# pingooio/pingoo

Hardware: AMD Instinct MI355X
Metric: requests/sec matched (whole node), 1k-rule WAF (higher is better)
Workload: dtype u8

## Files before the change

pingoo_amd/csrc/confirm.hip:

```cpp
#include <hip/hip_runtime.h>

#include <algorithm>

#include "confirm.h"
#include "hitrec.h"
#include "kernels.h"
#include "wave.h"

namespace pwaf {

__global__ __launch_bounds__(256) void confirm_plan_kernel(ConfirmTableDev b, uint32_t *plan ) {
    __shared__ uint32_t part[256];
    const uint32_t t = threadIdx.x;
    uint32_t items = 0;
    if (t < b.count) {
        const ConfirmArgs *pa = &b.c[t];
        const bool dense = pa->dense_flag != nullptr && *pa->dense_flag > pa->dense_thresh;
        items = dense ? 0u : (min(*pa->pair_count, pa->pair_cap) + kConfirmThreads - 1) / kConfirmThreads;
    }
    part[t] = items;
    __syncthreads();
    for (uint32_t d = 1; d < 256; d <<= 1) {
        const uint32_t v = t >= d ? part[t - d] : 0u;
        __syncthreads();
        part[t] += v;
        __syncthreads();
    }
    if (t < b.count) plan[t] = part[t] - items;
    if (t == 0) plan[b.count] = part[255];
}

__device__ __noinline__ void merge_atom(PoolEntry *pool, uint32_t *pool_count, uint32_t *status, uint32_t pool_cap, uint32_t *rec, uint32_t atom) {
    auto rmw_read = [](uint32_t *p) { return atomicOr(p, 0u); };
    auto publish = [&](uint32_t idx, uint32_t at, uint32_t next) {
        const uint32_t t0 = atomicExch(&pool[idx].atom, at), t1 = atomicExch(&pool[idx].next, next);
        asm volatile("" ::"v"(t0), "v"(t1));
    };
    uint32_t old = rmw_read(rec);
    for (;;) {
        uint32_t upd;
        const uint32_t x = atom + 1u;
        if (!(old & REC_OVERFLOW)) {
            const uint32_t a0 = old & 0x7FFFu, a1 = (old >> 15) & 0x7FFFu;
            if (a0 == x || a1 == x) return;
            if (a0 == 0u) upd = old | x;
            else if (a1 == 0u) upd = old | (x << 15);
            else {
                const uint32_t idx = atomicAdd(pool_count, 3u);
                if (idx + 3u > pool_cap) { atomicOr(status, 1u); return; }
                publish(idx, a0 - 1u, kNone);
                publish(idx + 1u, a1 - 1u, idx);
                publish(idx + 2u, atom, idx + 1u);
                upd = REC_OVERFLOW | (idx + 2u);
            }
        } else {
            const uint32_t head = old & ~REC_OVERFLOW;
            for (uint32_t i = head; i != kNone; i = rmw_read(&pool[i].next))
                if (rmw_read(&pool[i].atom) == atom) return;
            const uint32_t idx = atomicAdd(pool_count, 1u);
            if (idx >= pool_cap) { atomicOr(status, 1u); return; }
            publish(idx, atom, head);
            upd = REC_OVERFLOW | idx;
        }
        const uint32_t seen = atomicCAS(rec, old, upd);
        if (seen == old) return;
        old = seen;
    }
}

__global__ __launch_bounds__(kConfirmThreads, 8) void confirm_kernel(ConfirmTableDev b, const uint32_t *plan) {
    __shared__ uint32_t head[kFilterEntries], ftab[kFilterEntries];
    __shared__ uint32_t pool[kConfirmPoolBytes / 4];
    constexpr uint32_t kConfirmQueue = 1024;
    __shared__ uint32_t app_cnt, app_base, app_queue[kConfirmQueue];
    __builtin_amdgcn_s_setprio(3);
    if (threadIdx.x == 0) app_cnt = 0;
    const uint32_t total = plan[b.count];
    const uint32_t it0 = (uint32_t)((uint64_t)total * blockIdx.x / gridDim.x), it1 = (uint32_t)((uint64_t)total * (blockIdx.x + 1) / gridDim.x);
    for (uint32_t it = it0; it < it1;) {
        uint32_t ps = 0;
        for (uint32_t lo = 0, hi = b.count; lo + 1 < hi;) {
            const uint32_t mid = (lo + hi) >> 1;
            if (plan[mid] <= it) lo = mid;
            else hi = mid;
            ps = lo;
        }
        const uint32_t first_item = plan[ps], it_end = min(it1, plan[ps + 1]);
        const ConfirmArgs a = load_descriptor(&b.c[ps]);
        __syncthreads();
        {
            const uint4 *sh = reinterpret_cast<const uint4 *>(a.c_head), *sf = reinterpret_cast<const uint4 *>(a.ftable);
            constexpr uint32_t kPer = kFilterEntries / 4 / kConfirmThreads;
            uint4 vh[kPer], vf[kPer];
#pragma unroll
            for (uint32_t q = 0; q < kPer; q++) { vh[q] = sh[q * kConfirmThreads + threadIdx.x]; vf[q] = sf[q * kConfirmThreads + threadIdx.x]; }
#pragma unroll
            for (uint32_t q = 0; q < kPer; q++) {
                reinterpret_cast<uint4 *>(head)[q * kConfirmThreads + threadIdx.x] = vh[q];
                reinterpret_cast<uint4 *>(ftab)[q * kConfirmThreads + threadIdx.x] = vf[q];
            }
        }
        const uint32_t e_words = a.n_entries * 3u, b_words = a.n_bytes / 4u, c_words = a.n_class_words;
        const bool in_lds = confirm_tables_fit(a.n_entries, a.n_bytes, a.n_class_words);
        const ConfirmEntry *t_entries = a.c_entries;
        const uint8_t *t_bytes = a.c_bytes;
        const uint32_t *t_classes = a.c_classes;
        if (in_lds) {
            const uint32_t *se = reinterpret_cast<const uint32_t *>(a.c_entries), *sb = reinterpret_cast<const uint32_t *>(a.c_bytes);
            for (uint32_t k = threadIdx.x; k < e_words; k += kConfirmThreads) pool[k] = se[k];
            for (uint32_t k = threadIdx.x; k < b_words; k += kConfirmThreads) pool[e_words + k] = sb[k];
            for (uint32_t k = threadIdx.x; k < c_words; k += kConfirmThreads) pool[e_words + b_words + k] = a.c_classes[k];
            t_entries = reinterpret_cast<const ConfirmEntry *>(pool);
            t_bytes = reinterpret_cast<const uint8_t *>(pool + e_words);
            t_classes = pool + e_words + b_words;
        }
        __syncthreads();
        const ConfirmView cv{nullptr, t_entries, t_bytes, t_classes, a.mul, a.stride, a.init};
        const uint32_t n_p = min(*a.pair_count, a.pair_cap);
        auto pair_of = [&](const uint32_t item) -> uint2 {
            const uint32_t k = (item - first_item) * kConfirmThreads + threadIdx.x;
            return (item < it_end && k < n_p) ? a.pairs[k] : make_uint2(kNone, 0u);
        };
        uint2 pr_next = pair_of(it), pr_after = pair_of(it + 1u);
        uint32_t fs_next = 0u, fe_next = 0u;
        ConfirmBytes tb_next{};
        if (pr_next.x != kNone) {
            confirm_load64(reinterpret_cast<const uint8_t *>(a.off + pr_next.x), fs_next, fe_next);
            tb_next = confirm_chunk_bytes(a.data, pr_next.y, a.total + PWAF_ARENA_PAD);
        }
        for (; it < it_end; it++) {
            const uint2 pr = pr_next;
            const bool live = pr.x != kNone;
            uint32_t r = live ? pr.x : 0u;
            uint32_t fs = fs_next, fe = fe_next;
            const ConfirmBytes tb = tb_next;
            pr_next = pr_after;
            if (pr_next.x != kNone) {
                confirm_load64(reinterpret_cast<const uint8_t *>(a.off + pr_next.x), fs_next, fe_next);
                tb_next = confirm_chunk_bytes(a.data, pr_next.y, a.total + PWAF_ARENA_PAD);
            }
            pr_after = pair_of(it + 2u);
            ConfirmChunk ch{0u, 0ull};
            if (live) ch = confirm_windows_of(cv, tb, 0u, 0xFFFFFFFFu, pr.y, [&](const uint32_t bin) { return ftab[bin]; });
            uint32_t mask = ch.mask, cnt = 0, j = 0, e0 = 0, pos = 0, widx = 0;
            bool walk = false;
            auto settle = [&](const uint32_t rq, const uint32_t need_lits, const bool wk, const bool aggregated) -> bool {
                bool w2 = wk;
                if (need_lits & a.shared_bits) w2 = true;
                const uint32_t direct = need_lits & ~a.shared_bits;
                if (direct) enqueue_mask_once(a.gate_lists, a.gate_count, a.n, rq, direct, a.enq_bits, a.enq_words);
                if (!w2 || a.walk_list == nullptr) return false;
                const uint32_t bit = 1u << (rq & 31u);
                if (atomicOr(&a.walk_bits[rq >> 5], bit) & bit) return false;
                atomicOr(&a.valid_bits[rq >> 5], bit);
                if (aggregated) return true;
                a.walk_list[atomicAdd(a.walk_count, 1u)] = rq;
                return false;
            };
            uint32_t need = 0;
            for (;;) {
                if (__ballot(j < cnt || mask != 0u) == 0) break;
                while (j >= cnt && mask != 0u) {
                    const uint32_t k = (uint32_t)__builtin_ctz(mask);
                    mask &= mask - 1u;
                    pos = pr.y * 16u + k;
                    const uint32_t bin = confirm_bin_of(ch, widx++, a.data, pos, a.mul);
                    while (pos >= fe && r + 1u < a.n) {
                        settle(r, need, walk, false);
                        need = 0;
                        walk = false;
                        r++;
                        fs = fe;
                        fe = a.off[r + 1];
                    }
                    if (pos >= fe) continue;
                    const uint32_t hd = head[bin];
                    e0 = hd & 0xFFFFFu;
                    cnt = hd >> 20;
                    j = 0;
                }
                if (j < cnt) {
                    const uint32_t res = in_lds ? confirm_entry<3>(t_entries, t_bytes, t_classes, e0 + j, a.data, fs, fe, pos)
                                                : confirm_entry<1>(t_entries, t_bytes, t_classes, e0 + j, a.data, fs, fe, pos);
                    j++;
                    if (res == 2u) {
                        walk = true;
                    } else if (res & 1u) {
                        const uint32_t atom = res >> 8;
                        merge_atom(a.pool, a.pool_count, a.status, a.pool_cap, a.rec + r, atom);
                        atomicOr(&a.valid_bits[r >> 5], 1u << (r & 31u));
                        if (a.colmask_local != nullptr) need |= a.colmask_local[atom];
                    }
                }
            }
            const bool append = live && settle(r, need, walk, true);
            if (append) {
                const uint32_t slot = atomicAdd(&app_cnt, 1u);
                if (slot < kConfirmQueue) app_queue[slot] = r;
                else a.walk_list[atomicAdd(a.walk_count, 1u)] = r;
            }
        }
        __syncthreads();
        {
            const uint32_t queued = min(app_cnt, kConfirmQueue);
            if (threadIdx.x == 0 && queued != 0) app_base = atomicAdd(a.walk_count, queued);
            __syncthreads();
            for (uint32_t k = threadIdx.x; k < queued; k += kConfirmThreads) a.walk_list[app_base + k] = app_queue[k];
            __syncthreads();
            if (threadIdx.x == 0) app_cnt = 0;
        }
    }
}

int launch_confirm(const ConfirmArgs *host, uint32_t count, const ConfirmArgs *dev, uint32_t *plan, uint32_t n_cus, void *stream) {
    if (count == 0 || host[0].n == 0) return 0;
    if (count > 256) return (int)hipErrorInvalidValue;
    ConfirmTableDev b{dev, count};
    hipLaunchKernelGGL(confirm_plan_kernel, dim3(1), dim3(256), 0, (hipStream_t)stream, b, plan);
    hipError_t e = hipGetLastError();
    if (e != hipSuccess) return (int)e;
    uint64_t max_items = 0;
    for (uint32_t k = 0; k < count; k++) max_items += ((uint64_t)host[k].pair_cap + kConfirmThreads - 1) / kConfirmThreads;
    const uint32_t blocks = (uint32_t)std::min<uint64_t>(max_items, (uint64_t)std::max(1u, n_cus) * 2u);
    const uint32_t *cplan = plan;
    hipLaunchKernelGGL(confirm_kernel, dim3(blocks), dim3(kConfirmThreads), 0, (hipStream_t)stream, b, cplan);
    return (int)hipGetLastError();
}

}
```

pingoo_amd/csrc/engine.cpp:

```cpp
#include "dirtable.h"
#include "engine_impl.h"
#include "georec.h"

using namespace pwaf;

namespace {

Switches read_switches() {
    Switches s;
#ifdef PWAF_PROFILING
    const auto set = [](const char *name) { return getenv(name) != nullptr; };
    s.sync_each = set("PWAF_SYNC_EACH");
    if (set("PWAF_DEBUG_SKIP")) s.debug_skip = (uint32_t)strtoul(getenv("PWAF_DEBUG_SKIP"), nullptr, 0);
    s.attr_prio = set("PWAF_ATTR_PRIO");
    s.placement = set("PWAF_PLACEMENT") ? atoi(getenv("PWAF_PLACEMENT")) : set("PWAF_ATTR_INLINE") ? 1 : set("PWAF_ATTR_EARLY") ? 3 : 2;
    s.skip_attr = set("PWAF_SKIP_ATTR");
    s.skip_ipres = set("PWAF_SKIP_IPRES") || s.skip_attr;
    if (set("PWAF_LIST_SHAPE")) s.list_shape = (long)(uint32_t)atoi(getenv("PWAF_LIST_SHAPE"));
    if (set("PWAF_FILTER_DEBUG_SKIP")) s.filter_debug_skip = (uint32_t)atoi(getenv("PWAF_FILTER_DEBUG_SKIP"));
    s.attr_after_compact = set("PWAF_ATTR_AFTER_COMPACT");
    s.dump_counts = set("PWAF_DUMP_COUNTS");
    s.skip_identity = set("PWAF_SKIP_IDENTITY");
    s.side_priority_high = set("PWAF_SIDE_PRIORITY_HIGH");
    s.no_packed_staging = set("PWAF_NO_PACKED_STAGING");
#endif
    return s;
}

int upload_tables(pwaf_engine *e, const TablePlan &t) {
    const Program &P = *e->prog.p;
    int rc = PWAF_OK;
    const auto up = [&](DevBuf &buf, const auto &vec) { if (!rc) rc = upload(buf, vec); };
    static_cast<PlanShape &>(*e) = t;
    for (int var = 0; var < 2; var++) {
        up(e->iu_vals[var], t.iu_vals[var]);
        up(e->iu_masks[var], t.iu_masks[var]);
    }
    up(e->bit_atoms, t.bit_col);
    up(e->num_atoms, t.cmp_atoms);
    up(e->lazy_atoms, t.lazy_atoms);
    up(e->lits, t.lits);
    up(e->trig_off, t.trig_off);
    up(e->trig_rules, t.trig_rules);
    up(e->always_rules, t.always);
    up(e->country_luts, t.cc_masks);
    up(e->rules, P.rules);
    if (!t.rules_unrouted.empty()) up(e->rules_unrouted, t.rules_unrouted);
    up(e->set_masks, P.set_masks);
    up(e->ip_root4, P.ipset_trie.root4);
    up(e->ip_root6, P.ipset_trie.root6);
    up(e->ip_nodes, P.ipset_trie.nodes);
    up(e->class_rows, t.class_rows);
    up(e->geo_root4, t.geo_root4);
    up(e->geo_root6, t.geo_root6);
    up(e->geo_nodes, t.geo_nodes);
    up(e->leaf_root, std::vector<uint32_t>(65536, TRIE_LEAF));
    up(e->geo_leaf_root, std::vector<uint32_t>(65536, TRIE_LEAF | t.geo_default));
    if (P.n_residual) {
        up(e->residual_blob, P.residual_blob);
        up(e->residual_errors, std::vector<unsigned long long>(P.n_residual, 0ull));
        if (P.has_geo && P.residual_needs_geo) {
            const std::vector<uint32_t> leaf0(65536, TRIE_LEAF);
            up(e->geo_rec_root4, P.geo_trie.root4.empty() ? leaf0 : P.geo_trie.root4);
            up(e->geo_rec_root6, P.geo_trie.root6.empty() ? leaf0 : P.geo_trie.root6);
            up(e->geo_rec_nodes, P.geo_trie.nodes);
            up(e->geo_recs, P.geo_recs);
        }
    }
    return rc;
}

int upload_flat(FlatDev &d, const FlatImage &m) {
    int rc = PWAF_OK;
    const auto up = [&](DevBuf &buf, const auto &vec, size_t pad = 0) { if (!rc) rc = upload(buf, vec, pad); };
    static_cast<FlatShape &>(d) = m;
    up(d.flat, m.flat, 16);
    up(d.delta, m.delta, 16);
    up(d.flat_classmap, m.classmap);
    up(d.emit_off, m.emit_off);
    up(d.emit_list, m.emit_list);
    up(d.end_off, m.end_off);
    up(d.end_list, m.end_list);
    return rc;
}
int upload_group(pwaf_engine *e, size_t k, const TuneOut *T) {
    const Program &P = *e->prog.p;
    const DfaGroup &g = P.groups[k];
    DevGroup &d = e->groups[k];
    int rc;
    ScanImage m;
    if ((rc = build_device_group(g, P.lds_hot_budget, m, T ? &T->visits[k] : nullptr, T ? &T->class_freq[k] : nullptr))) return rc;
    static_cast<ScanShape &>(d) = m;
    if ((rc = upload(d.tab, m.tab, 16)) || (rc = upload(d.classmap, m.classmap)) || (rc = upload(d.special, m.special)) || (rc = upload(d.list_off, m.list_off)) ||
        (rc = upload(d.list, m.list)))
        return rc;
    FlatImage fm, rm;
    const uint32_t lds[2] = {flat_lds_bytes(false), flat_lds_bytes(true)};
    build_flat_images(g, d.filter, lds, T, k, fm, rm);
    if ((rc = upload_flat(d.fl, fm)) || !g.rtier) return rc;
    return upload_flat(d.rt, rm);
}

int assign_lists(pwaf_engine *e) {
    const Program &P = *e->prog.p;
    std::vector<GroupFilter> filters;
    for (const DevGroup &d : e->groups) filters.push_back(d.filter);
    PassPlan plan;
    plan_passes(P, filters, e->mean_len, e->residual_jit.function != nullptr, switches().skip_identity, plan);
    static_cast<PassShape &>(*e) = plan;
    std::vector<FlatShape> full, rtier;
    for (const DevGroup &d : e->groups) {
        full.push_back(d.fl);
        rtier.push_back(d.rt);
    }
    plan_list_scans(plan.roles, full, rtier, !(P.flags & PWAF_OPT_NO_DENSE_SWITCH), switches().skip_identity, switches().list_shape, e->list_plan);
    int rc = PWAF_OK;
    const auto up = [&](DevBuf &buf, const auto &vec) { if (!rc) rc = upload(buf, vec); };
    for (size_t k = 0; k < e->groups.size(); k++) {
        DevGroup &d = e->groups[k];
        static_cast<PassRole &>(d) = plan.roles[k];
        if (!d.filtered) continue;
        up(d.ftable, d.filter.table);
        if (!d.confirm) continue;
        const ConfirmTable &ct = d.filter.confirm;
        up(d.c_head, ct.head);
        up(d.c_entries, ct.entries);
        up(d.c_bytes, ct.bytes);
        up(d.c_classes, ct.classes);
    }
    if (!plan.short_atoms.empty()) up(e->short_atoms, plan.short_atoms);
    up(e->pass_table, plan.pass_table);
    up(e->colmask, plan.colmask);
    return rc;
}

}

namespace pwaf {

const Switches &switches() {
    static const Switches sw = read_switches();
    return sw;
}

void set_trie_args(const pwaf_engine *e, VerdictArgs &v) {
    const Program &P = *e->prog.p;
    const uint32_t *leaf = (const uint32_t *)e->leaf_root.p;
    v.ip_root4 = P.ipset_trie.root4.empty() ? leaf : (const uint32_t *)e->ip_root4.p;
    v.ip_root6 = P.ipset_trie.root6.empty() ? leaf : (const uint32_t *)e->ip_root6.p;
    v.ip_nodes = (const uint32_t *)e->ip_nodes.p;
    v.set_masks = (const uint32_t *)e->set_masks.p;
    v.set_words = P.set_words;
    v.n_ip_lists = P.n_ip_lists;
    const uint32_t *geo_leaf = (const uint32_t *)e->geo_leaf_root.p;
    v.geo_root4 = P.geo_trie.root4.empty() ? geo_leaf : (const uint32_t *)e->geo_root4.p;
    v.geo_root6 = P.geo_trie.root6.empty() ? geo_leaf : (const uint32_t *)e->geo_root6.p;
    v.geo_nodes = (const uint32_t *)e->geo_nodes.p;
    v.has_geo = P.has_geo ? 1u : 0u;
    v.dir24 = (const uint32_t *)e->dir24.p;
    v.dir_chunks = (const uint32_t *)e->dir_chunks.p;
    v.dir_vals = (const uint32_t *)e->dir_vals.p;
    v.dir_esc = (const uint2 *)e->dir_esc.p;
    v.dir_summary = (const uint32_t *)e->dir_summary.p;
    v.dir_sum_shift = e->dir_sum_shift;
    v.dir_common = e->dir_common;
    v.dir_coarse = (const uint32_t *)e->dir_coarse.p;
    v.dir_coarse_shift = e->dir_coarse_shift;
    v.dir_coarse_bytes = e->dir_coarse_bytes;
    v.class_rows = (const uint32_t *)e->class_rows.p;
    v.class_words = e->class_words;
    v.acmp_words = e->acmp_words;
    v.geo_default = e->geo_default;
// ... 360 lines not shown
```

pingoo_amd/csrc/engine_impl.h:

```cpp
#pragma once
#include <hip/hip_runtime_api.h>

#include <cstdio>
#include <algorithm>
#include <cstring>
#include <memory>
#include <mutex>
#include <string>
#include <vector>

#include "kernels.h"
#include "program_handle.h"
#include "scanplan.h"
#include "staging.h"
#include "tableplan.h"

#define HIP_TRY(expr)                                                                                              \
    do {                                                                                                           \
        hipError_t _e = (expr);                                                                                    \
        if (_e != hipSuccess) return pwaf::fail(PWAF_E_DEVICE, std::string(#expr) + ": " + hipGetErrorString(_e)); \
    } while (0)

#pragma GCC visibility push(hidden)
namespace pwaf {

struct Switches {
    bool sync_each = false;
    uint32_t debug_skip = 0;
    bool attr_prio = false;
    int placement = 2;
    bool skip_ipres = false;
    bool skip_attr = false;
    long list_shape = -1;
    uint32_t filter_debug_skip = 0;
    bool attr_after_compact = false;
    bool dump_counts = false;
    bool skip_identity = false;
    bool side_priority_high = false;
    bool no_packed_staging = false;
};
const Switches &switches();

struct DevBuf {
    void *p = nullptr;
    size_t cap = 0;
    DevBuf() = default;
    DevBuf(const DevBuf &) = delete;
    DevBuf &operator=(const DevBuf &) = delete;
    DevBuf(DevBuf &&o) noexcept : p(o.p), cap(o.cap) { o.p = nullptr; o.cap = 0; }
    DevBuf &operator=(DevBuf &&o) noexcept {
        if (this != &o) { release(); p = o.p; cap = o.cap; o.p = nullptr; o.cap = 0; }
        return *this;
    }
    ~DevBuf() { release(); }
    int reserve(size_t bytes) {
        if (bytes <= cap) return PWAF_OK;
        if (p) (void)hipFree(p);
        p = nullptr;
        cap = 0;
        size_t want = bytes + bytes / 8 + 256;
        hipError_t e = hipMalloc(&p, want);
        if (e != hipSuccess) return fail(PWAF_E_NOMEM, std::string("hipMalloc failed: ") + hipGetErrorString(e));
        cap = want;
        return PWAF_OK;
    }
    void release() {
        if (p) (void)hipFree(p);
        p = nullptr;
        cap = 0;
    }
};

struct PinBuf {
    void *p = nullptr;
    size_t cap = 0;
    PinBuf() = default;
    PinBuf(const PinBuf &) = delete;
    PinBuf &operator=(const PinBuf &) = delete;
    PinBuf(PinBuf &&o) noexcept : p(o.p), cap(o.cap) { o.p = nullptr; o.cap = 0; }
    PinBuf &operator=(PinBuf &&o) noexcept {
        if (this != &o) { release(); p = o.p; cap = o.cap; o.p = nullptr; o.cap = 0; }
        return *this;
    }
    ~PinBuf() { release(); }
    int reserve(size_t bytes) {
        if (bytes <= cap) return PWAF_OK;
        if (p) (void)hipHostFree(p);
        p = nullptr;
        cap = 0;
        size_t want = bytes + bytes / 4 + 4096;
        hipError_t e = hipHostMalloc(&p, want, hipHostMallocPortable);
        if (e != hipSuccess) return fail(PWAF_E_NOMEM, std::string("hipHostMalloc failed: ") + hipGetErrorString(e));
        cap = want;
        return PWAF_OK;
    }
    void release() {
        if (p) (void)hipHostFree(p);
        p = nullptr;
        cap = 0;
    }
};

template <class T>
int upload(DevBuf &b, const std::vector<T> &v, size_t pad_bytes = 0) {
    size_t bytes = v.size() * sizeof(T);
    int rc = b.reserve(bytes + pad_bytes + 16);
    if (rc) return rc;
    if (bytes) HIP_TRY(hipMemcpy(b.p, v.data(), bytes, hipMemcpyHostToDevice));
    if (pad_bytes + 16) HIP_TRY(hipMemset((char *)b.p + bytes, 0, pad_bytes + 16));
    return PWAF_OK;
}

struct FlatDev : FlatShape {
    DevBuf flat, flat_classmap, emit_off, emit_list, end_off, end_list, delta;
};

struct DevGroup : ScanShape, PassRole {
    DevBuf tab, classmap, special, list_off, list;
    uint32_t chunks = 1;
    GroupFilter filter;
    DevBuf ftable;
    FlatDev fl, rt;
    DevBuf c_head, c_entries, c_bytes, c_classes;
};

}

struct Scratch {
    using DevBuf = pwaf::DevBuf;
    using PinBuf = pwaf::PinBuf;
    std::mutex mu;
    hipStream_t stream = nullptr, side = nullptr;
    hipEvent_t ev_fork = nullptr, ev_join = nullptr, done = nullptr;
    bool used = false;
    hipStream_t last = nullptr;
    bool last_own = false;
    DevBuf status;
    uint64_t pool_entries = 0;
    struct View { void *p = nullptr; };
    View res_cols;
    bool retry = false;
    DevBuf err_sink;
    DevBuf ipres;
    DevBuf rec, pool, gate_lists, attr;
    DevBuf verdict_spill;
    DevBuf res_words;
    DevBuf zero_block;
    View ctrl, cand_bits, visit_bits, walk_bits;
    DevBuf chunk_bits, cand_cnt;
    DevBuf need;
    DevBuf pairs;
    DevBuf zero_off;
    static constexpr uint32_t kArgSlots = 8;
    DevBuf args;
    PinBuf arg_slot[kArgSlots];
    hipEvent_t arg_ev[kArgSlots] = {};
    bool arg_pending[kArgSlots] = {};
    uint32_t arg_next = 0;
    std::vector<DevBuf> stage_field_data, stage_field_off;
    DevBuf stage_ip, stage_v6, stage_port, stage_flags, stage_asn, stage_country, stage_out, stage_counts;
    DevBuf stage_route;
    DevBuf stage_hits, stage_hit_counts;
    DevBuf stage_geo;
    PinBuf pin_in, pin_out, pin_status;
    DevBuf packed;
    DevBuf rec_meta, rec_cols;
    PinBuf rec_pin, rec_back;
    int ensure(bool own_stream) {
        if (!side) {
            int least = 0, greatest = 0;
            (void)hipDeviceGetStreamPriorityRange(&least, &greatest);
            if (pwaf::switches().side_priority_high) least = greatest;
            if (hipStreamCreateWithPriority(&side, hipStreamNonBlocking, least) != hipSuccess || hipEventCreateWithFlags(&ev_fork, hipEventDisableTiming) != hipSuccess ||
                hipEventCreateWithFlags(&ev_join, hipEventDisableTiming) != hipSuccess || hipEventCreateWithFlags(&done, hipEventDisableTiming) != hipSuccess)
                return pwaf::fail(PWAF_E_DEVICE, "hipStreamCreate / hipEventCreate failed");
            for (hipEvent_t &ev : arg_ev)
                if (hipEventCreateWithFlags(&ev, hipEventDisableTiming) != hipSuccess) return pwaf::fail(PWAF_E_DEVICE, "hipEventCreate failed");
        }
        if (own_stream && !stream && hipStreamCreateWithFlags(&stream, hipStreamNonBlocking) != hipSuccess) return pwaf::fail(PWAF_E_DEVICE, "hipStreamCreate failed");
        return PWAF_OK;
    }
    ~Scratch() {
        for (hipEvent_t ev : arg_ev)
            if (ev) (void)hipEventDestroy(ev);
        if (stream) (void)hipStreamDestroy(stream);
        if (side) (void)hipStreamDestroy(side);
        for (hipEvent_t ev : {ev_fork, ev_join, done})
// ... 163 lines not shown
```

pingoo_amd/csrc/kernels.h:

```cpp
#pragma once
#include <cstdint>
#include <string>
#include <vector>

#include "program.h"
#include "scanplan.h"
#include "verdictplan.h"

namespace pwaf {

static constexpr int kMaxPasses = 250;
static constexpr int kVerdictPre = 12;
static constexpr uint32_t kDirChunkWords = 32;

static constexpr uint32_t REC_OVERFLOW = 0x80000000u;
struct PoolEntry {
    uint32_t atom;
    uint32_t next;
};

struct ScanArgs {
    const uint8_t *data;
    const uint32_t *off;
    uint32_t n;
    const uint16_t *tab;
    const uint8_t *classmap;
    const uint8_t *umap;
    uint32_t ill_class;
    const SpecialCell *special;
    const uint32_t *list_off;
    const uint16_t *list;
    uint32_t n_states, stride, n_classes, n_hot;
    uint32_t start_emit;
    uint32_t emit_base, special_base;
    uint32_t n_cus;
    uint32_t chunks;
    uint32_t *rec;
    PoolEntry *pool;
    uint32_t *pool_count;
    uint32_t pool_cap;
    uint32_t *status;
    const uint32_t *colmask_local;
    uint32_t n_local;
    uint32_t *gate_lists;
    uint32_t *gate_count;
};

static constexpr uint32_t kListWalks = 1;
struct ListScanArgs {
    const uint8_t *data;
    const uint32_t *off;
    uint32_t n;
    const uint16_t *flat;
    const uint8_t *classmap;
    const uint8_t *umap;
    uint32_t ill_class;
    uint32_t n_classes;
    uint32_t n_hot;
    const uint64_t *delta;
    uint32_t n_delta;
    const uint32_t *emit_off;
    const uint16_t *emit_list;
    const uint32_t *end_off;
    const uint16_t *end_list;
    uint32_t *rec;
    PoolEntry *pool;
    uint32_t *pool_count;
    uint32_t pool_cap;
    uint32_t *status;
    const uint32_t *colmask_local;
    uint32_t n_local;
    uint32_t *gate_lists;
    uint32_t *gate_count;
    uint32_t *enq_bits;
    uint32_t enq_words;
    uint32_t behind_filter;
    const uint32_t *req_list;
    const uint32_t *n_list;
    uint32_t *visited;
    uint32_t *need_out;
    uint32_t shared_bits;
    const uint32_t *need_in;
    uint32_t need_bit;
    uint32_t merge_rec;
    uint32_t n_cus;
    const uint32_t *dense_flag;
    uint32_t dense_thresh;
    uint32_t dense_mode;
};
struct ListOf {
    const uint32_t *req_list;
    uint32_t n_l;
};

struct ConfirmArgs {
    const uint8_t *data;
    const uint32_t *off;
    uint32_t n;
    uint32_t total;
    const uint2 *pairs;
    const uint32_t *pair_count;
    uint32_t pair_cap;
    uint32_t mul, stride, init;
    const uint32_t *ftable;
    const uint32_t *c_head;
    const ConfirmEntry *c_entries;
    const uint8_t *c_bytes;
    const uint32_t *c_classes;
    uint32_t n_entries, n_bytes, n_class_words;
    uint32_t *rec;
    uint32_t *valid_bits;
    uint32_t *walk_bits;
    uint32_t *walk_list;
    uint32_t *walk_count;
    PoolEntry *pool;
    uint32_t *pool_count;
    uint32_t pool_cap;
    uint32_t *status;
    const uint32_t *colmask_local;
    uint32_t n_local;
    uint32_t *gate_lists;
    uint32_t *gate_count;
    uint32_t *enq_bits;
    uint32_t enq_words;
    uint32_t shared_bits;
    const uint32_t *dense_flag;
    uint32_t dense_thresh;
};
static constexpr uint32_t kConfirmThreads = 1024;
static constexpr uint32_t kConfirmPoolBytes = 40 * 1024;
constexpr uint32_t confirm_table_bytes(const size_t pool_bytes) { return (uint32_t)pool_bytes & ~3u; }
constexpr bool confirm_tables_fit(const uint32_t n_entries, const uint32_t n_bytes, const uint32_t n_class_words) {
    return (uint64_t)n_entries * 3u + n_bytes / 4u + n_class_words <= kConfirmPoolBytes / 4;
}
struct ConfirmTableDev {
    const ConfirmArgs *c;
    uint32_t count;
};
int launch_confirm(const ConfirmArgs *host, uint32_t count, const ConfirmArgs *dev, uint32_t *plan, uint32_t n_cus, void *stream);

static constexpr uint32_t kStreamSlab = 128 * 1024;
static constexpr uint32_t kStreamIter = 4096;
static constexpr uint32_t kFilterWaves = 4;
static constexpr uint32_t kCompactWords = 2048;
struct FilterArgs {
    const uint8_t *data;
    const uint32_t *off;
    uint32_t n;
    uint32_t total;
    uint32_t slab0;
    uint32_t init;
    uint32_t mul;
    uint32_t stride;
    const uint32_t *table;
    uint32_t n_heads;
    uint32_t head_w[2][4];
    uint32_t head_m[2][4];
    uint32_t head_len[2];
    uint32_t head_code[2];
    uint32_t *rec;
    uint32_t *chunk_bits;
    uint32_t *sub_count;
    uint32_t *bitmap;
    uint32_t *block_count;
    uint32_t *list;
    uint32_t *list_count;
    uint2 *pairs;
    uint32_t *pair_count;
    uint32_t pair_cap;
    uint32_t *pair_base;
    const uint32_t *dense_flag;
    uint32_t dense_thresh;
    uint32_t first_block;
    uint32_t debug;
};
int upload_args_block(const void *host_pinned, void *dev, size_t bytes, void *zero , size_t zero_bytes, void *stream);
struct FilterTable {
    const FilterArgs *f;
    uint32_t count;
};
struct FilterMix {
    const FilterArgs *f1, *f2;
    uint32_t count1, count2, blocks1, blocks2;
};
int launch_filter(const FilterArgs *host1, uint32_t count1, const FilterArgs *dev1, const FilterArgs *host2, uint32_t count2, const FilterArgs *dev2, void *stream);
int launch_resolve(const FilterArgs *host, uint32_t count, const FilterArgs *dev, void *stream);
int launch_compact(const FilterArgs *host, uint32_t count, const FilterArgs *dev, void *stream);
int configure_kernels(int device);
int configure_scan_kernels();
int configure_filter_kernels();
int configure_verdict_kernels();

struct FcmpArgs {
    const uint8_t *data[kMaxFcmpFields];
    const uint32_t *off[kMaxFcmpFields];
    uint32_t atoms[kMaxFcmpAtoms];
    uint32_t n, n_atoms;
    uint32_t *rec;
    PoolEntry *pool;
    uint32_t *pool_count;
    uint32_t pool_cap;
    uint32_t *status;
};
int launch_fcmp(const FcmpArgs &a, void *stream);
struct ResidualArgs {
    const uint8_t *const *data;
    const uint32_t *const *off;
    const uint8_t *blob;
    uint32_t n, n_rules;
    const uint8_t *ip;
    const uint8_t *ip_is_v6;
    const uint16_t *port;
    const uint32_t *asn;
    const uint16_t *country;
    uint32_t has_geo;
    const uint32_t *geo_root4, *geo_root6, *geo_nodes;
    const GeoRec *geo_recs;
    uint32_t *rec;
    PoolEntry *pool;
    uint32_t *pool_count;
    uint32_t pool_cap;
    uint32_t *status;
    unsigned long long *rule_errors;
};
int launch_residual(const ResidualArgs &a, void *stream);
struct ResidualJitArgs {
    const uint8_t *const *data;
    const uint32_t *const *off;
    const uint8_t *blob;
    uint32_t n, n_rules;
    const uint8_t *ip;
    const uint8_t *ip_is_v6;
    const uint16_t *port;
    const uint32_t *asn;
    const uint16_t *country;
    uint32_t has_geo, pad;
    const uint32_t *geo_root4, *geo_root6, *geo_nodes;
    const GeoRec *geo_recs;
    uint32_t *match_words;
    unsigned long long *rule_errors;
};
struct JitKernel {
    void *module = nullptr, *function = nullptr;
};
static constexpr uint32_t kMaxJitRules = 256;
bool rvm_specialize(const uint8_t *blob, size_t len, std::string &out, std::string &why);
bool rvm_jit_program(const uint8_t *blob, size_t len, std::string &out, std::string &why);
bool rtc_compile(const std::string &source, const std::string &arch, std::vector<char> &code, std::string &why);
bool jit_load(const std::vector<char> &code, JitKernel &out, std::string &why);
void jit_release(JitKernel &k);
int launch_residual_jit(const JitKernel &k, const ResidualJitArgs &a, uint32_t n_cus, void *stream);
struct ColPtrChunk {
    const void *p[2 * (PWAF_N_FIELDS + kMaxHeaders)];
    uint32_t count;
};
struct VerdictArgs {
    uint32_t n, n_groups;
    uint32_t debug_skip;
    uint32_t force_global_tables;
    uint32_t sparse_mode;
    uint32_t v_cap;
    unsigned long long *spill;
    const uint32_t *off[PWAF_N_FIELDS];
    const uint8_t *ip;
    const uint8_t *ip_is_v6;
    const uint16_t *port;
    const uint8_t *flags;
    const uint32_t *asn;
    const uint16_t *country;
    uint32_t n_passes;
    const uint32_t *rec;
    const PassInfo *passes;
    const uint32_t *res_match;
    uint32_t res_words, res_base;
    const uint32_t *cand_bits, *visit_bits;
    uint32_t bit_words;
    const uint32_t *hoff[kMaxHeaderLens];
    const ShortAtom *short_atoms;
    uint32_t n_short;
    const uint8_t *short_data;
    const uint32_t *short_off;
    uint32_t n_hlen;
    const PoolEntry *pool;
    uint32_t n_cols;
    const CmpAtomDev *cmp;
    uint32_t n_cmp;
    uint32_t cmp_vars;
    const CmpAtomDev *lazy;
    uint32_t n_lazy;
    uint32_t lazy_var[4], n_lazy_var;
    const uint32_t *bit_col;
    const int64_t *iu_vals[2];
// ... 78 lines not shown
```

pingoo_amd/csrc/pipeline.cpp:

```cpp
#include <type_traits>

#include "engine_impl.h"
#include "georec.h"
#include "lscan_split.h"

using namespace pwaf;

namespace {

uint32_t slab_count(uint32_t total, uint32_t slab0) { return (uint32_t)(((uint64_t)total + kStreamSlab - 1) / kStreamSlab) - slab0; }
uint32_t slabs_of(const FilterArgs &f) { return slab_count(f.total, f.slab0); }
uint32_t pair_cap_of(uint32_t slabs, uint32_t n) { return (uint32_t)std::min<uint64_t>(0xFFFFFFF0u, (uint64_t)slabs * (kStreamSlab / 16) + n + 64); }

struct ArgSlotMark {
    Scratch &S;
    hipStream_t stream;
    int slot = -1;
    int record() {
        if (slot < 0) return PWAF_OK;
        const int k = slot;
        slot = -1;
        S.arg_pending[k] = true;
        HIP_TRY(hipEventRecord(S.arg_ev[k], stream));
        return PWAF_OK;
// ... 161 lines not shown
        v.gpairs = (uint4 *)S.attr.p;
        v.ghdr = (uint32_t *)((char *)S.attr.p + ((size_t)n_groups * pair_stride + 64) * 16);
        v.pair_stride = pair_stride;
        v.attr_blocks = e->n_cus;
        v.pool = (const PoolEntry *)S.pool.p;
        v.cmp = (const CmpAtomDev *)e->num_atoms.p;
        v.n_cmp = e->n_cmp_atoms;
        v.cmp_vars = e->cmp_vars;
        v.lazy = (const CmpAtomDev *)e->lazy_atoms.p;
        v.n_lazy = e->n_lazy;
        v.n_lazy_var = (uint32_t)e->lazy_vars.size();
        for (size_t k = 0; k < e->lazy_vars.size(); k++) v.lazy_var[k] = e->lazy_vars[k];
        v.n_short = e->n_short;
        v.short_atoms = (const ShortAtom *)e->short_atoms.p;
        if (e->n_short) {
            v.short_data = cols[(size_t)e->short_field].data;
            v.short_off = cols[(size_t)e->short_field].offsets;
        }
        v.n_trig = e->n_trig;
        v.n_lits = (uint32_t)P.lits.size();
        v.bit_col = (const uint32_t *)e->bit_atoms.p;
        v.trig_off = (const uint32_t *)e->trig_off.p;
        v.trig_rules = (const uint16_t *)e->trig_rules.p;
        v.always_rules = (const uint32_t *)e->always_rules.p;
        for (int var = 0; var < 2; var++) {
            v.iu_vals[var] = (const int64_t *)e->iu_vals[var].p;
            v.iu_masks[var] = (const uint32_t *)e->iu_masks[var].p;
            v.iu_n[var] = e->iu_n[var];
            v.iu_words[var] = e->iu_words[var];
        }
        v.country_masks = (const uint32_t *)e->country_luts.p;
        v.cc_words = e->cc_words;
        v.rules = (const DevRule *)e->rules.p;
        v.n_rules = (uint32_t)P.rules.size();
        v.lits = (const uint32_t *)e->lits.p;
        set_trie_args(e, v);
        if ((rc = S.ipres.reserve((size_t)n * (v.ipres_packed ? 4 : 8) + 64))) return rc;
        v.ipres = (uint32_t *)S.ipres.p;
        v.out = d_out;
        v.counts = (unsigned long long *)d_counts;
        v.match_idx = d_match_idx;
        v.n_matches = d_n_matches;
        return PWAF_OK;
    }

    int zero_head_records() {
        for (size_t k = 0; k < e->groups.size(); k++) {
            const DevGroup &d = e->groups[k];
            if (!d.filtered || d.filter.heads.empty()) continue;
            if (slab_count(col_bytes[d.field], slab0_of(d.field)) != 0 && !(sw.filter_debug_skip & 4u)) continue;
            HIP_TRY(hipMemsetAsync((uint32_t *)S.rec.p + k * (size_t)n, 0, (size_t)n * 4, stream));
        }
        return PWAF_OK;
    }


    template <class Launch>
    int timed(const char *name, uint64_t bytes, const char *what, Launch &&launch, hipStream_t side = nullptr) {
        const int rc = prof.begin(side);
        if (rc) return rc;
        const int he = launch();
        if (he) return fail(PWAF_E_DEVICE, std::string(what) + " launch failed: " + hipGetErrorString((hipError_t)he));
        return prof.end(name, bytes, side);
    }

    template <class Launch>
    int side_stage(hipStream_t q, const char *name, uint64_t code, const char *what, Launch &&launch) {
        const hipStream_t side = q != stream ? q : nullptr;
        const int rc = timed(name, code, what, launch, side);
        if (rc) return rc;
        if (side) HIP_TRY(hipEventRecord(S.ev_join, q));
        return PWAF_OK;
    }
    int ipres_stage(hipStream_t q) {
        if (ipres_launched) return PWAF_OK;
        ipres_launched = true;
        if (q != stream) {
            HIP_TRY(hipEventRecord(S.ev_fork, stream));
            HIP_TRY(hipStreamWaitEvent(q, S.ev_fork, 0));
        }
        const int rc = side_stage(q, "ipres", 0xFAu, "ipres kernel", [&] { return sw.skip_ipres ? (int)hipMemsetAsync(v.ipres, 0, (size_t)n * (v.ipres_packed ? 4 : 8), q) : launch_ipres(v, q); });
        if (rc || !d_geo) return rc;
        GeoRecArgs ga{};
        set_georec_args(e, ga);
        ga.ip = db.ip;
        ga.ip_is_v6 = db.ip_is_v6;
        ga.asn = db.asn;
        ga.country = db.country;
        ga.n = n;
        ga.out = (uint2 *)d_geo;
        return side_stage(q, "georec", 25ull * n, "georec kernel", [&] { return launch_georec(ga, q); });
    }
    int attr_stage(hipStream_t q) {
        if (attr_launched) return PWAF_OK;
        attr_launched = true;
        if (q == stream && sw.placement == 0) HIP_TRY(hipStreamWaitEvent(stream, S.ev_join, 0));
        return side_stage(q, "attr", 0xFEu, "attribute kernel", [&] { return sw.skip_attr ? (int)hipMemsetAsync(v.ghdr, 0, (size_t)n_groups * 4, q) : launch_attr(v, q); });
    }
    int attr_at_start() {
        int rc;
        if (sw.placement == 0) return ipres_stage(S.side);
        if (sw.placement == 3) return (rc = ipres_stage(S.side)) ? rc : attr_stage(S.side);
        return PWAF_OK;
    }
    int attr_after_filter() {
        int rc;
        switch (sw.placement) {
        case 0: return attr_stage(stream);
        case 1: return (rc = ipres_stage(stream)) ? rc : attr_stage(stream);
        case 2: return (rc = ipres_stage(S.side)) ? rc : attr_stage(S.side);
        default: return PWAF_OK;
        }
    }
    int join_side() {
        if (sw.placement >= 2) HIP_TRY(hipStreamWaitEvent(stream, S.ev_join, 0));
        return PWAF_OK;
    }

    int launch_plain_scans() {
        static const char *fn[5] = {"host", "url", "path", "method", "user_agent"};
        for (size_t gi = 0; gi < e->groups.size(); gi++) {
            const DevGroup &d = e->groups[gi];
            if (d.gate >= 0 || d.identity || d.short_lit) continue;
            const ScanArgs a = scan_args(gi);
            char nm[48];
            if (d.field < PWAF_N_FIELDS) snprintf(nm, sizeof nm, "scan_%s_g%zu", fn[d.field], gi);
            else snprintf(nm, sizeof nm, "scan_hdr%u_g%zu", d.field - PWAF_N_FIELDS, gi);
            prof.streaming = true;
            const int rc = timed(nm, (uint64_t)col_bytes[d.field] + 4ull * (n + 1), "scan kernel", [&] { return launch_scan(a, stream); });
            prof.streaming = false;
            if (rc) return rc;
        }
        return PWAF_OK;
    }

    int launch_filter_stage() {
        prof.streaming = true;
        const int rc = timed(by_stride[1].empty() ? "filter_s1" : by_stride[0].empty() ? "filter_s2" : "filter_mix", alg_bytes[1] + alg_bytes[2], "filter kernel", [&] {
            return launch_filter(by_stride[0].data(), (uint32_t)by_stride[0].size(), d_s1, by_stride[1].data(), (uint32_t)by_stride[1].size(), d_s2, stream);
        });
        prof.streaming = false;
        return rc;
    }
    int launch_resolve_stage() {
        bool any_list = false;
        for (const DevGroup &d : e->groups) any_list = any_list || (d.filtered && !d.confirm);
        return timed("resolve+compact", 0xFCu, "resolve / compact kernel", [&] {
            const int he = launch_resolve(fall.data(), (uint32_t)fall.size(), d_all, stream);
            return !he && any_list ? launch_compact(fall.data(), (uint32_t)fall.size(), d_all, stream) : he;
        });
    }
    int launch_confirm_stage() {
        if (call.empty()) return PWAF_OK;
        return timed("confirm", 0xF8u, "confirm kernel", [&] { return launch_confirm(call.data(), (uint32_t)call.size(), d_c, c_plan, e->n_cus, stream); });
    }
    int launch_list_scans() {
        uint32_t *plan_at = l_plan;
        for (int phase = 0; phase < 2; phase++) {
            uint32_t first = 0;
            for (const uint32_t cnt : e->lscan_launches[phase]) {
                char nm[48];
                snprintf(nm, sizeof nm, "lscan_x%u", cnt);
                const int rc = timed(nm, 0xFDu, "gated scan kernel", [&] { return launch_scan_gated(la[phase].data() + first, cnt, d_la[phase] + first, plan_at, lshapes[phase], stream); });
                if (rc) return rc;
                plan_at += 2 * cnt + 1;
                first += cnt;
            }
        }
        return PWAF_OK;
    }
    int launch_fcmp_stage() {
        if (P.fcmp.empty()) return PWAF_OK;
        FcmpArgs fa{};
        std::vector<uint32_t> slots;
        for (size_t k = 0; k < P.fcmp.size(); k++) {
            uint32_t sl[2];
            const uint32_t fld[2] = {P.fcmp[k].a, P.fcmp[k].b};
            for (int q = 0; q < 2; q++) {
                size_t at = std::find(slots.begin(), slots.end(), fld[q]) - slots.begin();
                if (at == slots.size()) slots.push_back(fld[q]);
                sl[q] = (uint32_t)at;
            }
            fa.atoms[k] = P.fcmp[k].op | (sl[0] << 8) | (sl[1] << 16);
        }
        for (size_t q = 0; q < slots.size() && q < kMaxFcmpFields; q++) {
            fa.data[q] = cols[slots[q]].data;
            fa.off[q] = cols[slots[q]].offsets;
        }
        fa.n = n;
        fa.n_atoms = (uint32_t)P.fcmp.size();
        fa.rec = (uint32_t *)S.rec.p + e->groups.size() * (size_t)n;
        set_pool(fa);
        return timed("fcmp", 0xFBu, "field comparison kernel", [&] { return launch_fcmp(fa, stream); });
    }
    template <class Args>
    int residual_inputs(Args &a) {
        a.data = (const uint8_t *const *)S.res_cols.p;
        a.off = (const uint32_t *const *)((const char *)S.res_cols.p + (size_t)e->n_fields * 8);
        a.blob = (const uint8_t *)e->residual_blob.p;
        a.n = n;
        a.n_rules = P.n_residual;
        a.ip = db.ip;
        a.ip_is_v6 = db.ip_is_v6;
        a.port = db.port;
        a.asn = db.asn;
        a.country = db.country;
        a.has_geo = (P.has_geo && P.residual_needs_geo) ? 1u : 0u;
        a.geo_root4 = (const uint32_t *)e->geo_rec_root4.p;
        a.geo_root6 = (const uint32_t *)e->geo_rec_root6.p;
        a.geo_nodes = (const uint32_t *)e->geo_rec_nodes.p;
        a.geo_recs = (const GeoRec *)e->geo_recs.p;
        a.rule_errors = (unsigned long long *)e->residual_errors.p;
        if (S.retry) {
            const int rc = S.err_sink.reserve((size_t)P.n_residual * 8);
            if (rc) return rc;
            a.rule_errors = (unsigned long long *)S.err_sink.p;
        }
        return PWAF_OK;
    }
    int launch_residual_stage() {
        if (!P.n_residual) return PWAF_OK;
        int rc;
        if (e->residual_jit.function) {
            ResidualJitArgs ja{};
            if ((rc = residual_inputs(ja))) return rc;
            ja.match_words = (uint32_t *)S.res_words.p;
            return timed("residual_jit", 0xF9u, "specialized residual kernel", [&] { return launch_residual_jit(e->residual_jit, ja, e->n_cus, stream); });
        }
        ResidualArgs ra{};
        if ((rc = residual_inputs(ra))) return rc;
        ra.rec = (uint32_t *)S.rec.p + (size_t)residual_pass * n;
        set_pool(ra);
        return timed("residual", 0xF9u, "residual kernel", [&] { return launch_residual(ra, stream); });
    }
    int launch_verdict_stage() { return timed("verdict", 0xFFu, "verdict kernel", [&] { return launch_verdict(v, stream); }); }
    int dump_counts() {
        std::vector<uint32_t> cw(ctrl_words);
        HIP_TRY(hipStreamSynchronize(stream));
        HIP_TRY(hipMemcpy(cw.data(), S.ctrl.p, 4 * ctrl_words, hipMemcpyDeviceToHost));
        fprintf(stderr, "[pwaf] n %u pool %u status %u |", n, cw[0], cw[1]);
        for (size_t k = 0; k < e->groups.size(); k++) {
            const DevGroup &d = e->groups[k];
            if (d.gate >= 0) fprintf(stderr, " pass %zu field %u %s list %u", k, d.field, d.filtered ? (d.confirm ? "confirm" : "filtered") : "gap", cw[2 + (size_t)d.gate]);
        }
        for (uint32_t k = 0; k < e->n_filtered; k++) fprintf(stderr, " pairs[%u] %u", k, cw[2 + n_slots + k]);
        fprintf(stderr, "\n");
        return PWAF_OK;
    }


    template <class Args>
    void set_pool(Args &a) const {
        a.pool = (PoolEntry *)S.pool.p;
        a.pool_count = (uint32_t *)S.ctrl.p;
        a.pool_cap = pool_cap;
        a.status = status_word;
    }
    bool feeds_gates(size_t gi) const { return e->n_gap && e->owns_factors[gi]; }
    template <class Args>
    void set_gate_feed(Args &a, const DevGroup &d) const {
        a.colmask_local = (const uint32_t *)e->colmask.p + d.atom_base;
        a.n_local = d.n_local;
        a.gate_lists = (uint32_t *)S.gate_lists.p;
        a.gate_count = (uint32_t *)S.ctrl.p + 2;
        if constexpr (!std::is_same<Args, ScanArgs>::value) {
            a.enq_bits = (uint32_t *)S.visit_bits.p;
            a.enq_words = bit_words;
        }
    }

    ScanArgs scan_args(size_t gi) const {
        const DevGroup &d = e->groups[gi];
        ScanArgs a{};
        if (feeds_gates(gi)) set_gate_feed(a, d);
        a.data = cols[d.field].data;
        a.off = cols[d.field].offsets;
        a.n = n;
        a.tab = (const uint16_t *)d.tab.p;
        a.classmap = (const uint8_t *)d.classmap.p;
        a.umap = d.scalar_mode ? (const uint8_t *)d.classmap.p + kUmapAt : nullptr;
        a.ill_class = d.ill_class;
        a.special = (const SpecialCell *)d.special.p;
        a.list_off = (const uint32_t *)d.list_off.p;
        a.list = (const uint16_t *)d.list.p;
        a.start_emit = d.start_emit;
        a.emit_base = d.emit_base;
        a.n_cus = e->n_cus;
        a.chunks = d.chunks;
        a.special_base = d.special_base;
        a.n_states = d.n_states;
        a.stride = d.stride;
        a.n_classes = d.n_classes;
        a.n_hot = d.n_hot;
        a.rec = (uint32_t *)S.rec.p + gi * (size_t)n;
        set_pool(a);
        return a;
    }

    int learn_arena_sizes() {
        bool ask = false;
        for (const DevGroup &d : e->groups)
            if (d.filtered && !col_known[d.field]) {
                HIP_TRY(hipMemcpyAsync(&col_bytes[d.field], cols[d.field].offsets + n, 4, hipMemcpyDeviceToHost, stream));
                ask = true;
            }
        if (ask) HIP_TRY(hipStreamSynchronize(stream));
        return PWAF_OK;
// ... 357 lines not shown
```

Baseline: 7.592 billion.

## Batch confirmed atoms per record in registers before atomic merge into rec

Instead of calling the noinline merge_atom with several global atomics for every confirmed hit, each lane keeps up to two distinct atom ids for the current record in a register and flushes them with one CAS-from-zero, falling back to the full merge only when the record is already populated. The window index is also packed into the upper bits of the mask and the entry loop uses a start/end cursor, which saves registers. The aim is to cut global atomic traffic and call overhead on the hot confirm path. It adds profiling-only debug switches that can skip confirm work, and it changes the order in which atoms are published to the record.

```diff
diff --git a/pingoo_amd/csrc/confirm.hip b/pingoo_amd/csrc/confirm.hip
--- a/pingoo_amd/csrc/confirm.hip
+++ b/pingoo_amd/csrc/confirm.hip
@@ -30,24 +30,23 @@
     if (t == 0) plan[b.count] = part[255];
 }
 
-__device__ __noinline__ void merge_atom(PoolEntry *pool, uint32_t *pool_count, uint32_t *status, uint32_t pool_cap, uint32_t *rec, uint32_t atom) {
+__device__ __forceinline__ uint32_t merge_atom(PoolEntry *pool, uint32_t *pool_count, uint32_t *status, uint32_t pool_cap, uint32_t *rec, uint32_t atom, uint32_t old) {
     auto rmw_read = [](uint32_t *p) { return atomicOr(p, 0u); };
     auto publish = [&](uint32_t idx, uint32_t at, uint32_t next) {
         const uint32_t t0 = atomicExch(&pool[idx].atom, at), t1 = atomicExch(&pool[idx].next, next);
         asm volatile("" ::"v"(t0), "v"(t1));
     };
-    uint32_t old = rmw_read(rec);
     for (;;) {
         uint32_t upd;
         const uint32_t x = atom + 1u;
         if (!(old & REC_OVERFLOW)) {
             const uint32_t a0 = old & 0x7FFFu, a1 = (old >> 15) & 0x7FFFu;
-            if (a0 == x || a1 == x) return;
+            if (a0 == x || a1 == x) return old;
             if (a0 == 0u) upd = old | x;
             else if (a1 == 0u) upd = old | (x << 15);
             else {
                 const uint32_t idx = atomicAdd(pool_count, 3u);
-                if (idx + 3u > pool_cap) { atomicOr(status, 1u); return; }
+                if (idx + 3u > pool_cap) { atomicOr(status, 1u); return old; }
                 publish(idx, a0 - 1u, kNone);
                 publish(idx + 1u, a1 - 1u, idx);
                 publish(idx + 2u, atom, idx + 1u);
@@ -56,16 +55,34 @@
         } else {
             const uint32_t head = old & ~REC_OVERFLOW;
             for (uint32_t i = head; i != kNone; i = rmw_read(&pool[i].next))
-                if (rmw_read(&pool[i].atom) == atom) return;
+                if (rmw_read(&pool[i].atom) == atom) return old;
             const uint32_t idx = atomicAdd(pool_count, 1u);
-            if (idx >= pool_cap) { atomicOr(status, 1u); return; }
+            if (idx >= pool_cap) { atomicOr(status, 1u); return old; }
             publish(idx, atom, head);
             upd = REC_OVERFLOW | idx;
         }
         const uint32_t seen = atomicCAS(rec, old, upd);
-        if (seen == old) return;
+        if (seen == old) return upd;
         old = seen;
     }
+}
+__device__ __noinline__ void merge_kept(const ConfirmArgs *pa, uint32_t r, uint32_t kept, uint32_t seen) {
+    const uint32_t p0 = kept & 0x7FFFu, p1 = kept >> 15;
+    PoolEntry *const pool = pa->pool;
+    uint32_t *const pool_count = pa->pool_count, *const status = pa->status, *const rec = pa->rec + r;
+    const uint32_t pool_cap = pa->pool_cap;
+    seen = merge_atom(pool, pool_count, status, pool_cap, rec, p0 - 1u, seen);
+    if (p1 != 0u) merge_atom(pool, pool_count, status, pool_cap, rec, p1 - 1u, seen);
+}
+__device__ __noinline__ uint32_t merge_early(const ConfirmArgs *pa, uint32_t r, uint32_t kept) {
+    const uint32_t p0 = kept & 0x7FFFu, p1 = kept >> 15;
+    const uint32_t seen = atomicCAS(pa->rec + r, 0u, kept);
+    atomicOr(&pa->valid_bits[r >> 5], 1u << (r & 31u));
+    const uint32_t *const colmask_local = pa->colmask_local;
+    uint32_t need = 0;
+    if (colmask_local != nullptr) need = colmask_local[p0 - 1u] | (p1 != 0u ? colmask_local[p1 - 1u] : 0u);
+    if (seen != 0u) merge_kept(pa, r, kept, seen);
+    return need;
 }
 
 __global__ __launch_bounds__(kConfirmThreads, 8) void confirm_kernel(ConfirmTableDev b, const uint32_t *plan) {
@@ -142,7 +159,7 @@
             pr_after = pair_of(it + 2u);
             ConfirmChunk ch{0u, 0ull};
             if (live) ch = confirm_windows_of(cv, tb, 0u, 0xFFFFFFFFu, pr.y, [&](const uint32_t bin) { return ftab[bin]; });
-            uint32_t mask = ch.mask, cnt = 0, j = 0, e0 = 0, pos = 0, widx = 0;
+            uint32_t mask = ch.mask, e_at = 0, e_end = 0, pos = 0;
             bool walk = false;
             auto settle = [&](const uint32_t rq, const uint32_t need_lits, const bool wk, const bool aggregated) -> bool {
                 bool w2 = wk;
@@ -158,14 +175,26 @@
                 return false;
             };
             uint32_t need = 0;
+            uint32_t kept = 0;
+#ifdef PWAF_PROFILING
+            const bool merges = !(b.debug & 3u);
+#else
+            constexpr bool merges = true;
+#endif
+            auto merge_in_loop = [&]() {
+                if (kept != 0u && merges) need |= merge_early(&b.c[ps], r, kept);
+            };
             for (;;) {
-                if (__ballot(j < cnt || mask != 0u) == 0) break;
-                while (j >= cnt && mask != 0u) {
+                if (__ballot(e_at < e_end || (mask & 0xFFFFu) != 0u) == 0) break;
+                while (e_at >= e_end && (mask & 0xFFFFu) != 0u) {
                     const uint32_t k = (uint32_t)__builtin_ctz(mask);
-                    mask &= mask - 1u;
+                    const uint32_t widx = mask >> 16;
+                    mask = (mask & (mask - 1u)) + 0x10000u;
                     pos = pr.y * 16u + k;
-                    const uint32_t bin = confirm_bin_of(ch, widx++, a.data, pos, a.mul);
+                    const uint32_t bin = confirm_bin_of(ch, widx, a.data, pos, a.mul);
                     while (pos >= fe && r + 1u < a.n) {
+                        merge_in_loop();
+                        kept = 0u;
                         settle(r, need, walk, false);
                         need = 0;
                         walk = false;
@@ -175,23 +204,43 @@
                     }
                     if (pos >= fe) continue;
                     const uint32_t hd = head[bin];
-                    e0 = hd & 0xFFFFFu;
-                    cnt = hd >> 20;
-                    j = 0;
+                    e_at = hd & 0xFFFFFu;
+                    e_end = e_at + (hd >> 20);
                 }
-                if (j < cnt) {
-                    const uint32_t res = in_lds ? confirm_entry<3>(t_entries, t_bytes, t_classes, e0 + j, a.data, fs, fe, pos)
-                                                : confirm_entry<1>(t_entries, t_bytes, t_classes, e0 + j, a.data, fs, fe, pos);
-                    j++;
+                if (e_at < e_end) {
+                    const uint32_t res = in_lds ? confirm_entry<3>(t_entries, t_bytes, t_classes, e_at, a.data, fs, fe, pos)
+#ifdef PWAF_PROFILING
+                                   : (b.debug & 2u) ? 0u
+#endif
+                                                    : confirm_entry<1>(t_entries, t_bytes, t_classes, e_at, a.data, fs, fe, pos);
+                    e_at++;
                     if (res == 2u) {
                         walk = true;
                     } else if (res & 1u) {
-                        const uint32_t atom = res >> 8;
-                        merge_atom(a.pool, a.pool_count, a.status, a.pool_cap, a.rec + r, atom);
-                        atomicOr(&a.valid_bits[r >> 5], 1u << (r & 31u));
-                        if (a.colmask_local != nullptr) need |= a.colmask_local[atom];
+                        const uint32_t x = (res >> 8) + 1u;
+                        if (x != (kept & 0x7FFFu) && x != (kept >> 15)) {
+                            if (kept == 0u) kept = x;
+                            else if ((kept >> 15) == 0u) kept |= x << 15;
+                            else {
+                                merge_in_loop();
+                                kept = x;
+                            }
+                        }
                     }
                 }
+            }
+            if (kept != 0u && merges) {
+                const uint32_t seen = atomicCAS(a.rec + r, 0u, kept);
+                atomicOr(&a.valid_bits[r >> 5], 1u << (r & 31u));
+                if (a.colmask_local != nullptr) {
+                    need |= a.colmask_local[(kept & 0x7FFFu) - 1u];
+                    if ((kept >> 15) != 0u) need |= a.colmask_local[(kept >> 15) - 1u];
+                }
+#ifdef PWAF_PROFILING
+                if (b.debug & 4u) need = 0;
+                if (!(b.debug & 8u))
+#endif
+                if (seen != 0u) merge_kept(&b.c[ps], r, kept, seen);
             }
             const bool append = live && settle(r, need, walk, true);
             if (append) {
@@ -212,10 +261,10 @@
     }
 }
 
-int launch_confirm(const ConfirmArgs *host, uint32_t count, const ConfirmArgs *dev, uint32_t *plan, uint32_t n_cus, void *stream) {
+int launch_confirm(const ConfirmArgs *host, uint32_t count, const ConfirmArgs *dev, uint32_t *plan, uint32_t n_cus, void *stream, uint32_t debug) {
     if (count == 0 || host[0].n == 0) return 0;
     if (count > 256) return (int)hipErrorInvalidValue;
-    ConfirmTableDev b{dev, count};
+    ConfirmTableDev b{dev, count, debug};
     hipLaunchKernelGGL(confirm_plan_kernel, dim3(1), dim3(256), 0, (hipStream_t)stream, b, plan);
     hipError_t e = hipGetLastError();
     if (e != hipSuccess) return (int)e;
diff --git a/pingoo_amd/csrc/engine.cpp b/pingoo_amd/csrc/engine.cpp
--- a/pingoo_amd/csrc/engine.cpp
+++ b/pingoo_amd/csrc/engine.cpp
@@ -18,6 +18,7 @@
     s.skip_ipres = set("PWAF_SKIP_IPRES") || s.skip_attr;
     if (set("PWAF_LIST_SHAPE")) s.list_shape = (long)(uint32_t)atoi(getenv("PWAF_LIST_SHAPE"));
     if (set("PWAF_FILTER_DEBUG_SKIP")) s.filter_debug_skip = (uint32_t)atoi(getenv("PWAF_FILTER_DEBUG_SKIP"));
+    if (set("PWAF_CONFIRM_DEBUG_SKIP")) s.confirm_debug_skip = (uint32_t)atoi(getenv("PWAF_CONFIRM_DEBUG_SKIP"));
     s.attr_after_compact = set("PWAF_ATTR_AFTER_COMPACT");
     s.dump_counts = set("PWAF_DUMP_COUNTS");
     s.skip_identity = set("PWAF_SKIP_IDENTITY");
diff --git a/pingoo_amd/csrc/engine_impl.h b/pingoo_amd/csrc/engine_impl.h
--- a/pingoo_amd/csrc/engine_impl.h
+++ b/pingoo_amd/csrc/engine_impl.h
@@ -33,6 +33,7 @@
     bool skip_attr = false;
     long list_shape = -1;
     uint32_t filter_debug_skip = 0;
+    uint32_t confirm_debug_skip = 0;
     bool attr_after_compact = false;
     bool dump_counts = false;
     bool skip_identity = false;
diff --git a/pingoo_amd/csrc/kernels.h b/pingoo_amd/csrc/kernels.h
--- a/pingoo_amd/csrc/kernels.h
+++ b/pingoo_amd/csrc/kernels.h
@@ -136,8 +136,9 @@
 struct ConfirmTableDev {
     const ConfirmArgs *c;
     uint32_t count;
-};
-int launch_confirm(const ConfirmArgs *host, uint32_t count, const ConfirmArgs *dev, uint32_t *plan, uint32_t n_cus, void *stream);
+    uint32_t debug;
+};
+int launch_confirm(const ConfirmArgs *host, uint32_t count, const ConfirmArgs *dev, uint32_t *plan, uint32_t n_cus, void *stream, uint32_t debug = 0);
 
 static constexpr uint32_t kStreamSlab = 128 * 1024;
 static constexpr uint32_t kStreamIter = 4096;
diff --git a/pingoo_amd/csrc/pipeline.cpp b/pingoo_amd/csrc/pipeline.cpp
--- a/pingoo_amd/csrc/pipeline.cpp
+++ b/pingoo_amd/csrc/pipeline.cpp
@@ -337,7 +337,7 @@
     }
     int launch_confirm_stage() {
         if (call.empty()) return PWAF_OK;
-        return timed("confirm", 0xF8u, "confirm kernel", [&] { return launch_confirm(call.data(), (uint32_t)call.size(), d_c, c_plan, e->n_cus, stream); });
+        return timed("confirm", 0xF8u, "confirm kernel", [&] { return launch_confirm(call.data(), (uint32_t)call.size(), d_c, c_plan, e->n_cus, stream, sw.confirm_debug_skip); });
     }
     int launch_list_scans() {
         uint32_t *plan_at = l_plan;
```

Measured after the change: 7.652 billion (median of 6 runs). No clear change (+0.8%).
